# GoatWu/AdaLog

Measured on AMD Instinct MI355X. Metric: calib_images_per_sec, higher is better.
Workload: dtype bf16

## Files before the change

### adalog_amd/csrc/sorted_score.hip

```cpp
#include "common.h"
#include "fpcs_tail.h"
#include <stdlib.h>

namespace {

typedef double d2 __attribute__((ext_vector_type(2)));
constexpr int PB = 1024;

__device__ __forceinline__ double wave_sum_d(double v) {
#pragma unroll
    for (int o = 32; o > 0; o >>= 1) v += __shfl_xor(v, o);
    return v;
}

__global__ __launch_bounds__(256) void k_sp_blocksum(const float* __restrict__ sorted, int64_t n, int nb, d2* __restrict__ bsum) {
    __shared__ double sm[2][4];
    const int64_t seg = blockIdx.y, b = blockIdx.x;
    const float* x = sorted + seg * n;
    const int64_t i0 = b * PB + (int64_t)threadIdx.x * 4;
    double s1 = 0.0, s2 = 0.0;
#pragma unroll
    for (int e = 0; e < 4; ++e) {
        if (i0 + e < n) { const double v = (double)x[i0 + e]; s1 += v; s2 += v * v; }
    }
    s1 = wave_sum_d(s1); s2 = wave_sum_d(s2);
    const int w = threadIdx.x >> 6;
    if ((threadIdx.x & 63) == 0) { sm[0][w] = s1; sm[1][w] = s2; }
    __syncthreads();
    if (threadIdx.x == 0) {
        d2 o = {(sm[0][0] + sm[0][1]) + (sm[0][2] + sm[0][3]), (sm[1][0] + sm[1][1]) + (sm[1][2] + sm[1][3])};
        bsum[seg * nb + b] = o;
    }
}

__global__ __launch_bounds__(256) void k_sp_blockscan(d2* __restrict__ bsum, int nb) {
    __shared__ double sm[2][4];
    d2* p = bsum + (int64_t)blockIdx.x * nb;
    double c1 = 0.0, c2 = 0.0;
    const int lane = threadIdx.x & 63, w = threadIdx.x >> 6;
    for (int base = 0; base < nb; base += 256) {
        const int i = base + threadIdx.x;
        d2 v = {0.0, 0.0};
        if (i < nb) v = p[i];
        double a1 = v.x, a2 = v.y;
#pragma unroll
        for (int o = 1; o < 64; o <<= 1) {
            const double u1 = __shfl_up(a1, o), u2 = __shfl_up(a2, o);
            if (lane >= o) { a1 += u1; a2 += u2; }
        }
        if (lane == 63) { sm[0][w] = a1; sm[1][w] = a2; }
        __syncthreads();
        double o1 = c1, o2 = c2;
        for (int j = 0; j < w; ++j) { o1 += sm[0][j]; o2 += sm[1][j]; }
        const double t1 = ((sm[0][0] + sm[0][1]) + sm[0][2]) + sm[0][3], t2 = ((sm[1][0] + sm[1][1]) + sm[1][2]) + sm[1][3];
        if (i < nb) { d2 e = {o1 + a1 - v.x, o2 + a2 - v.y}; p[i] = e; }
        c1 += t1; c2 += t2;
        __syncthreads();
    }
}

__global__ __launch_bounds__(256) void k_sp_prefix(const float* __restrict__ sorted, int64_t n, int nb, const d2* __restrict__ bofs,
                                                   d2* __restrict__ prefix) {
    __shared__ double sm[2][4];
    const int64_t seg = blockIdx.y, b = blockIdx.x;
    const float* x = sorted + seg * n;
    d2* out = prefix + seg * (n + 1);
    const int64_t i0 = b * PB + (int64_t)threadIdx.x * 4;
    double v1[4], v2[4];
#pragma unroll
    for (int e = 0; e < 4; ++e) {
        const double v = (i0 + e < n) ? (double)x[i0 + e] : 0.0;
        v1[e] = v; v2[e] = v * v;
    }
    const double t1 = (v1[0] + v1[1]) + (v1[2] + v1[3]), t2 = (v2[0] + v2[1]) + (v2[2] + v2[3]);
    double a1 = t1, a2 = t2;
    const int lane = threadIdx.x & 63, w = threadIdx.x >> 6;
#pragma unroll
    for (int o = 1; o < 64; o <<= 1) {
        const double u1 = __shfl_up(a1, o), u2 = __shfl_up(a2, o);
        if (lane >= o) { a1 += u1; a2 += u2; }
    }
    if (lane == 63) { sm[0][w] = a1; sm[1][w] = a2; }
    __syncthreads();
    const d2 base = bofs[seg * nb + b];
    double o1 = base.x + (a1 - t1), o2 = base.y + (a2 - t2);
    for (int j = 0; j < w; ++j) { o1 += sm[0][j]; o2 += sm[1][j]; }
#pragma unroll
    for (int e = 0; e < 4; ++e) {
        if (i0 + e <= n) { d2 o = {o1, o2}; out[i0 + e] = o; }
        o1 += v1[e]; o2 += v2[e];
    }
    if (i0 + 4 == n) { d2 o = {o1, o2}; out[n] = o; }
}

template <int G>
__global__ __launch_bounds__(256) void k_score_sorted(const float* __restrict__ sorted, const d2* __restrict__ prefix, int64_t S,
                                                      int64_t n, const float* __restrict__ scale, const float* __restrict__ zp,
                                                      int P, float qmax, double norm, float* __restrict__ scores) {
    constexpr int GPB = 256 / G;
    __shared__ int64_t bnd[GPB][G + 1];
    __shared__ double red[256];
    const int gi = threadIdx.x / G, t = threadIdx.x % G;
    const int64_t pair = (int64_t)blockIdx.x * GPB + gi;
    const bool live = pair < (int64_t)P * S;
    const int64_t seg = live ? pair % S : 0;
    const float s = live ? scale[pair] : 1.0f, z = live ? zp[pair] : 0.0f;
    const float klo = ceilf(-z), khi = floorf(qmax - z);
    const float* x = sorted + seg * n;
    const d2* pf = prefix + seg * (n + 1);
    auto lower = [&](float target) {
        int64_t lo = 0, hi = n;
        while (lo < hi) {
            const int64_t mid = (lo + hi) >> 1;
            if (rintf(x[mid] / s) >= target) hi = mid; else lo = mid + 1;
        }
        return lo;
    };
    if (live) {
        bnd[gi][t] = lower(fminf(klo + (float)t, khi + 1.0f));
        if (t == 0) bnd[gi][G] = lower(khi + 1.0f);
    }
    __syncthreads();
    double acc = 0.0;
    if (live) {
        auto run = [&](int64_t a, int64_t b, float level) {
            if (b <= a) return 0.0;
            const float q = fminf(fmaxf(level + z, 0.0f), qmax);
            const double c = (double)((q - z) * s);
            const d2 pa = pf[a], pb = pf[b];
            return (pb.y - pa.y) - 2.0 * c * (pb.x - pa.x) + (double)(b - a) * c * c;
        };
        acc = run(bnd[gi][t], bnd[gi][t + 1], klo + (float)t);
        if (t == 0) acc += run(0, bnd[gi][0], klo - 1.0f) + run(bnd[gi][G], n, khi + 1.0f);
    }
    red[threadIdx.x] = acc;
    __syncthreads();
#pragma unroll
    for (int o = G / 2; o > 0; o >>= 1) {
        if (t < o) red[threadIdx.x] += red[threadIdx.x + o];
        __syncthreads();
    }
    if (live && t == 0) scores[pair] = (float)(-norm * red[threadIdx.x]);
}

size_t sort_temp_bytes(int64_t S, int64_t n) {
    const int64_t b = adalog_sort_workspace_bytes(S, n, 0);
    return (size_t)((b < 256 ? 256 : b) + 255) / 256 * 256;
}

}

extern "C" int64_t adalog_sorted_prefix_workspace_bytes(int64_t S, int64_t n) {
    if (S < 1 || n < 1 || S * n >= ((int64_t)1 << 31)) return -1;
    const int64_t nb = (n + PB - 1) / PB;
    return (int64_t)sort_temp_bytes(S, n) + ((S + 1) * 4 + 255) / 256 * 256 + S * nb * 16;
}

extern "C" int adalog_sorted_prefix_build(const float* x, int64_t S, int64_t n, float* sorted, double* prefix, void* workspace,
                                          int64_t workspace_bytes, void* stream) {
    ADALOG_ARG_CHECK(x && sorted && prefix && workspace && S >= 1 && n >= 1, "sorted_prefix_build: bad arguments");
    ADALOG_ARG_CHECK(S * n < ((int64_t)1 << 31), "sorted_prefix_build: more than 2^31 - 1 elements");
    ADALOG_ARG_CHECK(workspace_bytes >= adalog_sorted_prefix_workspace_bytes(S, n), "sorted_prefix_build: workspace too small");
    ADALOG_ARG_CHECK((((uintptr_t)workspace | (uintptr_t)prefix) & 15) == 0, "sorted_prefix_build: workspace / prefix must be 16-byte aligned");
    hipStream_t st = (hipStream_t)stream;
    size_t tb = sort_temp_bytes(S, n);
    uint8_t* ws = (uint8_t*)workspace;
    int* offs = (int*)(ws + tb);
    d2* bsum = (d2*)(ws + tb + ((S + 1) * 4 + 255) / 256 * 256);
    ADALOG_ARG_CHECK(((uintptr_t)workspace & 255) == 0 || n <= 8192, "sorted_prefix_build: workspace must be 256-byte aligned");
    {
        const int rc = adalog_sort_f32(x, S, n, sorted, nullptr, ws, (int64_t)tb, stream);
        if (rc) return rc;
    }
    const int nb = cdiv(n, PB);
    ADALOG_ARG_CHECK(S <= 65535, "sorted_prefix_build: more than 65535 segments");
    hipLaunchKernelGGL(k_sp_blocksum, dim3(nb, (unsigned)S), dim3(256), 0, st, sorted, n, nb, bsum);
    hipLaunchKernelGGL(k_sp_blockscan, dim3((unsigned)S), dim3(256), 0, st, bsum, nb);
    hipLaunchKernelGGL(k_sp_prefix, dim3(nb, (unsigned)S), dim3(256), 0, st, sorted, n, nb, bsum, (d2*)prefix);
    ADALOG_LAUNCH_CHECK("adalog_sorted_prefix_build");
    return 0;
}

extern "C" int adalog_score_self_sorted_tail(const float* sorted, const double* prefix, int64_t S, int64_t n, const float* scale,
                                             const float* zp, int P, int n_bits, double norm, float* scores,
                                             const adalog_fpcs_tail* tail, void* stream) {
    ADALOG_ARG_CHECK(sorted && prefix && scale && zp && scores && S >= 1 && n >= 1 && P >= 1, "score_self_sorted: bad arguments");
    ADALOG_ARG_CHECK(n_bits >= 1 && n_bits <= 8, "score_self_sorted: 1..8 bits");
    const char* why = fpcs::tail_problem(tail, P);
    ADALOG_ARG_CHECK(why == nullptr, why);
    const float qmax = (float)((1 << n_bits) - 1);
    const int G = 1 << n_bits;
    hipStream_t st = (hipStream_t)stream;
    const int64_t pairs = (int64_t)P * S;
    const int gpb = 256 / G;
    const int64_t blocks = (pairs + gpb - 1) / gpb;
    ADALOG_ARG_CHECK(blocks < ((int64_t)1 << 31), "score_self_sorted: grid too large");
    adalog_dispatch<1, 2, 3, 4, 5, 6, 7, 8>(n_bits, [&](auto nb) {
        return adalog_launch<k_score_sorted<(1 << decltype(nb)::value)>>("k_score_sorted", 0, (unsigned)blocks, 256, 0, st, sorted, (const d2*)prefix,
                                                                          S, n, scale, zp, P, qmax, norm, scores);
    });
    ADALOG_LAUNCH_CHECK("adalog_score_self_sorted");
    if (tail) return adalog_topk_next_tail(scores, P, (int)S, tail, nullptr, stream);
    return 0;
}

extern "C" int adalog_score_self_sorted(const float* sorted, const double* prefix, int64_t S, int64_t n, const float* scale,
                                        const float* zp, int P, int n_bits, double norm, float* scores, void* stream) {
    return adalog_score_self_sorted_tail(sorted, prefix, S, n, scale, zp, P, n_bits, norm, scores, nullptr, stream);
}
```

Baseline: 38.81.

## Stage sorted segments in LDS for binary-search scoring with segment/candidate planning

Adds a segment-tiled scoring kernel that copies one or more sorted segments into LDS and then evaluates many (scale, zero-point) candidates against them, so the binary-search probes hit shared memory instead of global memory. A host planner picks segments-per-block and candidates-per-block from the segment count, length and CU count, and falls back to the original kernel for long segments or when an env var disables it. The scoring body is factored into a shared device helper that is templated on index type so the LDS path can use 32-bit indices. This trades extra LDS staging and a larger dynamic shared allocation, which can lower occupancy, for far fewer scattered global loads.

```diff
diff --git a/adalog_amd/csrc/sorted_score.hip b/adalog_amd/csrc/sorted_score.hip
--- a/adalog_amd/csrc/sorted_score.hip
+++ b/adalog_amd/csrc/sorted_score.hip
@@ -93,26 +93,16 @@
     if (i0 + 4 == n) { d2 o = {o1, o2}; out[n] = o; }
 }
 
-template <int G>
-__global__ __launch_bounds__(256) void k_score_sorted(const float* __restrict__ sorted, const d2* __restrict__ prefix, int64_t S,
-                                                      int64_t n, const float* __restrict__ scale, const float* __restrict__ zp,
-                                                      int P, float qmax, double norm, float* __restrict__ scores) {
-    constexpr int GPB = 256 / G;
-    __shared__ int64_t bnd[GPB][G + 1];
-    __shared__ double red[256];
+template <int G, class I, class Probe>
+__device__ __forceinline__ void score_group(Probe probe, const d2* __restrict__ pf, int64_t n, bool live, int64_t pair, float s, float z,
+                                            float qmax, double norm, int64_t (*bnd)[G + 1], double* red, float* __restrict__ scores) {
     const int gi = threadIdx.x / G, t = threadIdx.x % G;
-    const int64_t pair = (int64_t)blockIdx.x * GPB + gi;
-    const bool live = pair < (int64_t)P * S;
-    const int64_t seg = live ? pair % S : 0;
-    const float s = live ? scale[pair] : 1.0f, z = live ? zp[pair] : 0.0f;
     const float klo = ceilf(-z), khi = floorf(qmax - z);
-    const float* x = sorted + seg * n;
-    const d2* pf = prefix + seg * (n + 1);
     auto lower = [&](float target) {
-        int64_t lo = 0, hi = n;
+        I lo = 0, hi = (I)n;
         while (lo < hi) {
-            const int64_t mid = (lo + hi) >> 1;
-            if (rintf(x[mid] / s) >= target) hi = mid; else lo = mid + 1;
+            const I mid = (lo + hi) >> 1;
+            if (rintf(probe(mid) / s) >= target) hi = mid; else lo = mid + 1;
         }
         return lo;
     };
@@ -141,6 +131,89 @@
         __syncthreads();
     }
     if (live && t == 0) scores[pair] = (float)(-norm * red[threadIdx.x]);
+}
+
+template <int G>
+__global__ __launch_bounds__(256) void k_score_sorted(const float* __restrict__ sorted, const d2* __restrict__ prefix, int64_t S,
+                                                      int64_t n, const float* __restrict__ scale, const float* __restrict__ zp,
+                                                      int P, float qmax, double norm, float* __restrict__ scores) {
+    constexpr int GPB = 256 / G;
+    __shared__ int64_t bnd[GPB][G + 1];
+    __shared__ double red[256];
+    const int gi = threadIdx.x / G;
+    const int64_t pair = (int64_t)blockIdx.x * GPB + gi;
+    const bool live = pair < (int64_t)P * S;
+    const int64_t seg = live ? pair % S : 0;
+    const float s = live ? scale[pair] : 1.0f, z = live ? zp[pair] : 0.0f;
+    const float* x = sorted + seg * n;
+    score_group<G, int64_t>([&](int64_t mid) { return x[mid]; }, prefix + seg * (n + 1), n, live, pair, s, z, qmax, norm, bnd, red, scores);
+}
+
+constexpr int SEG_MAX_FLOATS = 14 * 1024;
+extern __shared__ float4 lds_dyn[];
+template <int G>
+__global__ __launch_bounds__(256) void k_score_sorted_seg(const float* __restrict__ sorted, const d2* __restrict__ prefix, int S, int n,
+                                                          int spw, int cps, const float* __restrict__ scale, const float* __restrict__ zp,
+                                                          int P, float qmax, double norm, float* __restrict__ scores) {
+    constexpr int GPB = 256 / G;
+    __shared__ int64_t bnd[GPB][G + 1];
+    __shared__ double red[256];
+    const int seg0 = blockIdx.x * spw, ns = min(spw, S - seg0);
+    const int p0 = blockIdx.y * cps, np = min(cps, P - p0);
+    const float* src = sorted + (int64_t)seg0 * n;
+    const int total = ns * n;
+    const int head = min((int)((16 - ((uintptr_t)src & 15)) & 15) >> 2, total);
+    const int nvec = (total - head) >> 2, rest = head + 4 * nvec;
+    float* xs = (float*)lds_dyn + ((4 - head) & 3);
+    {
+        const float4* s4 = (const float4*)(src + head);
+        float4* d4 = (float4*)(xs + head);
+        for (int v = threadIdx.x; v < nvec; v += 256) d4[v] = s4[v];
+        if ((int)threadIdx.x < head) xs[threadIdx.x] = src[threadIdx.x];
+        if ((int)threadIdx.x < total - rest) xs[rest + threadIdx.x] = src[rest + threadIdx.x];
+    }
+    __syncthreads();
+    const int gi = threadIdx.x / G, items = ns * np;
+    for (int w0 = 0; w0 < items; w0 += GPB) {
+        const bool live = w0 + gi < items;
+        const int w = live ? w0 + gi : 0;
+        const int sl = w % ns, seg = seg0 + sl;
+        const int64_t pair = (int64_t)(p0 + w / ns) * S + seg;
+        const float s = live ? scale[pair] : 1.0f, z = live ? zp[pair] : 0.0f;
+        const float* x = xs + sl * n;
+        score_group<G, int>([&](int mid) { return x[mid]; }, prefix + (int64_t)seg * (n + 1), n, live, pair, s, z, qmax, norm, bnd, red, scores);
+    }
+}
+
+struct SortedPlan {
+    bool seg;
+    int spw, cps;
+};
+
+SortedPlan score_sorted_plan(int64_t S, int64_t n, int P, int n_bits) {
+    SortedPlan pl = {false, 1, P};
+    const char* e = getenv("ADALOG_SCORE_SORTED_LDS");
+    if ((e && atoi(e) == 0) || n > SEG_MAX_FLOATS || S >= ((int64_t)1 << 30)) return pl;
+    pl.seg = true;
+    const int gpb = 256 >> n_bits, passes = (P + gpb - 1) / gpb;
+    const int fit = (int)(160 * 1024 / (n * 4 + 5 * 1024));
+    const int64_t T = (int64_t)adalog_device_cus() * (fit < 8 ? fit : 8);
+    int ps = 1;
+    if (S >= 2 * T) {
+        const int64_t a = S / T, b = 3840 / n;
+        pl.spw = (int)(a < b ? a : b);
+        if (pl.spw < 1) pl.spw = 1;
+    } else if (n <= 2048) {
+        ps = passes < 65535 ? passes : 65535;
+    } else {
+        double best = 0.0;
+        for (int c = 1; c <= passes && c <= 16; ++c) {
+            const double cost = (double)((S * c + T - 1) / T) * ((double)n / 2048.0 + (double)((passes + c - 1) / c));
+            if (c == 1 || cost < best) { best = cost; ps = c; }
+        }
+    }
+    pl.cps = ((P + ps - 1) / ps + gpb - 1) / gpb * gpb;
+    return pl;
 }
 
 size_t sort_temp_bytes(int64_t S, int64_t n) {
@@ -189,16 +262,21 @@
     const char* why = fpcs::tail_problem(tail, P);
     ADALOG_ARG_CHECK(why == nullptr, why);
     const float qmax = (float)((1 << n_bits) - 1);
-    const int G = 1 << n_bits;
     hipStream_t st = (hipStream_t)stream;
-    const int64_t pairs = (int64_t)P * S;
-    const int gpb = 256 / G;
-    const int64_t blocks = (pairs + gpb - 1) / gpb;
-    ADALOG_ARG_CHECK(blocks < ((int64_t)1 << 31), "score_self_sorted: grid too large");
-    adalog_dispatch<1, 2, 3, 4, 5, 6, 7, 8>(n_bits, [&](auto nb) {
-        return adalog_launch<k_score_sorted<(1 << decltype(nb)::value)>>("k_score_sorted", 0, (unsigned)blocks, 256, 0, st, sorted, (const d2*)prefix,
-                                                                          S, n, scale, zp, P, qmax, norm, scores);
+    const SortedPlan pl = score_sorted_plan(S, n, P, n_bits);
+    const int gpb = 256 >> n_bits;
+    const int64_t blocks = ((int64_t)P * S + gpb - 1) / gpb;
+    ADALOG_ARG_CHECK(pl.seg || blocks < ((int64_t)1 << 31), "score_self_sorted: grid too large");
+    const int rc = adalog_dispatch<1, 2, 3, 4, 5, 6, 7, 8>(n_bits, [&](auto nb) {
+        constexpr int G = 1 << decltype(nb)::value;
+        if (pl.seg)
+            return adalog_launch<k_score_sorted_seg<G>>("k_score_sorted_seg", 0, dim3((unsigned)cdiv(S, pl.spw), (unsigned)cdiv(P, pl.cps)), 256,
+                                                        ((size_t)pl.spw * n + 3) * 4, st, sorted, (const d2*)prefix, (int)S, (int)n, pl.spw,
+                                                        pl.cps, scale, zp, P, qmax, norm, scores);
+        return adalog_launch<k_score_sorted<G>>("k_score_sorted", 0, (unsigned)blocks, 256, 0, st, sorted, (const d2*)prefix, S, n, scale, zp, P,
+                                                qmax, norm, scores);
     });
+    if (rc) return rc;
     ADALOG_LAUNCH_CHECK("adalog_score_self_sorted");
     if (tail) return adalog_topk_next_tail(scores, P, (int)S, tail, nullptr, stream);
     return 0;
```

New measurement: 39.31, median of 6. 1.3% higher.
